# Celebrandil/CudaSift

Hardware: AMD Instinct MI355X
Metric: 1920x1080 SIFT frames/sec (higher is better)
Workload: dtype f32

## Files before the change

cudasift_amd/csrc/common.hpp:

```cpp
#pragma once
#include <hip/hip_runtime.h>
#include <stdint.h>
#include <stddef.h>
#include "misift.h"

#define NUM_SCALES 5
#define NUM_BLURS  8
#define NUM_DOG    7
#define CNT_STRIDE 64
#define CNT_MAXPTS 17
#define CNT_CAND   20
#define CNT_CANDOVF 28
#define CNT_PTOVF  29
#define CNT_CHAINTMO 30
#define CNT_DET    32
#define CNT_DUP    40
#define CNT_SPARE_BLOCKS 9
#define CNT_BIG    48
#define CNT_TICKET 49
#define CNT_ORIDONE 50
#define CNT_FUSETMO 31

struct alignas(16) SiftPointD {
  float xpos, ypos, scale, sharpness, edgeness, orientation, score, ambiguity;
// ... 281 lines not shown
  unsigned int *d_counters;
  unsigned int *h_counters;
  int cap_frames;
  unsigned int *d_cand;
  size_t cand_cap;
  Detection *d_det;
  Detection *d_det_sorted;
  int descr_occ;
  int tile_descr, tile_orient;
  int bin_detections;
  int cap_det_frames, det_max_pts;
  float *d_own_scratch;
  size_t own_scratch_floats;
  int lds_pad_lpd, lds_pad_scan, lds_pad_orient, lds_pad_descr;
  float patch_reach;
  int fold_descr_tail;
  int descr_big_fallbacks;
  PendingBig pending_big;
  unsigned *d_refcap;
  size_t refcap_bytes;
  unsigned *d_capcnt;
  size_t capcnt_bytes;
  int refcap_limit;
  void *d_match_tmp;
  size_t match_tmp_bytes;
  int num_cus;
  int split_tail, in_capture;
  hipStream_t stream2;
  hipEvent_t ev_fork, ev_join;
  int *pack_counts, *pack_offsets;
  SiftPointD *pack_dst;
  int orient_blocks_per_cu;
  int point_blocks_per_cu;
  int strip_waves_per_cu, scan_waves_per_cu;
  int chain_max_frames;
  int chain_embed;
  unsigned chain_wait_ticks;
  int chain_fallbacks;
  int fuse_orient;
  unsigned fuse_wait_ticks;
  int fuse_fallbacks;
  int bin_min_frames;
  int small_frames;
  int lowpass_tile;
  int strip_rows_small;
  int scan_rows_small_coarse;
// ... 25 lines not shown
hipStream_t misift_ctx_result_stream(misift_ctx *ctx);
int misift_ensure_tmp(misift_ctx *ctx, size_t bytes);
int launch_refcap(misift_ctx *ctx, int w, int h, int nframes, int octave);
int launch_descr_big_pending(misift_ctx *ctx);
bool misift_tiny_call(int width, int height, int num_octaves);
int misift_extract_enqueue(misift_ctx *ctx, const void *d_imgs, int src_u8, int nframes, long long frame_stride,
                           int width, int height, int pitch, int num_octaves, float init_blur, float thresh,
                           float lowest_scale, int scale_up, float *d_scratch, SiftPointD *pts, int max_pts);
int misift_extract_sync(misift_ctx *ctx, const void *d_imgs, int src_u8, int nframes, long long frame_stride, int width,
                        int height, int pitch, int num_octaves, float init_blur, float thresh, float lowest_scale,
                        int scale_up, float *d_scratch, SiftPointD *pts, int max_pts, int *num_pts_out);
int launch_export_counts(misift_ctx *ctx, int nframes, int num_octaves, int max_pts, int *counts_out,
                         int *offsets_out);
int launch_pack_records(misift_ctx *ctx, const SiftPointD *pts, int max_pts, int nframes, const int *offsets,
                        SiftPointD *packed);

#define HIP_TRY(expr)                                                                        \
  do {                                                                                       \
    hipError_t e_ = (expr);                                                                  \
    if (e_ != hipSuccess) {                                                                  \
      misift_set_error("%s failed: %s (%s:%d)", #expr, hipGetErrorString(e_), __FILE__, __LINE__); \
      return MISIFT_EHIP;                                                                    \
    }                                                                                        \
  } while (0)

struct LaunchScope {
  misift_ctx *ctx;
  const char *name;
  LaunchScope(misift_ctx *c, const char *n);
  int finish();
// ... 21 lines not shown
int launch_dog_scan(misift_ctx *ctx, const float *base, const StripGeom &g, const LaplaceTaps &taps,
                      float thresh, int octave);
int launch_refine(misift_ctx *ctx, const float *dog, long long dog_frame_stride, const float *base,
                  long long base_frame_stride, const LaplaceTaps *taps, int w, int h, int pitch, int nframes,
                  float thresh, float edge_limit, float factor, float lowest_scale, float subsampling, int octave,
                  SiftPointD *pts, int max_pts);
int launch_orient(misift_ctx *ctx, const float *base, long long base_frame_stride, int w, int h, int pitch,
                  int nframes, int octave, SiftPointD *pts, int max_pts);
int launch_descr(misift_ctx *ctx, const float *base, long long base_frame_stride, int w, int h, int pitch,
                 int nframes, float subsampling, int octave, SiftPointD *pts, int max_pts);
int launch_rescale(misift_ctx *ctx, SiftPointD *pts, int npts, float scale);
int launch_rescale_batch(misift_ctx *ctx, SiftPointD *pts, int max_pts, int nframes, int num_octaves, float scale);
int launch_sort_segments(misift_ctx *ctx, SiftPointD *pts, int max_pts, int nframes, int num_octaves);
int launch_bin_detections(misift_ctx *ctx, const PyramidInfo &P, int max_pts);
int launch_renumber_dups(misift_ctx *ctx, const PyramidInfo &P, int max_pts);
int launch_orient_all(misift_ctx *ctx, const float *scratch, const PyramidInfo &P, SiftPointD *pts, int max_pts);
int launch_orient_descr_fused(misift_ctx *ctx, const float *scratch, const PyramidInfo &P, SiftPointD *pts, int max_pts);
int launch_descr_all(misift_ctx *ctx, const float *scratch, const PyramidInfo &P, SiftPointD *pts, int max_pts,
                     const int *pack_offsets, SiftPointD *pack_dst);
int launch_export_counts_staged(misift_ctx *ctx, int nframes, int num_octaves, int max_pts, int *counts_out,
                                int *offsets_out);
struct ScanAll;
struct ChainGeom;
int launch_dog_scan_all(misift_ctx *ctx, const float *scratch, const PyramidInfo &P, const LaplaceTaps *taps,
                        float thresh, int lev_begin, int lev_end, const ChainGeom *chain = nullptr,
                        const float *k5 = nullptr);
int make_chain_geom(ChainGeom *G, long long frame_stride, const int (*dims)[3], const long long *offs, int nlev, int tile);
int launch_refine_all(misift_ctx *ctx, const float *scratch, const PyramidInfo &P, const LaplaceTaps *taps,
                      float thresh, float edge_limit, float factor, int max_pts);
int launch_match(misift_ctx *ctx, SiftPointD *pts1, int row_begin, int row_count, const SiftPointD *pts2, int n2);
int launch_match_split(misift_ctx *ctx, SiftPointD *pts1, int row_begin, int row_count, const SiftPointD *pts2, int n2,
// ... 29 lines not shown
```

cudasift_amd/csrc/kernels_points.hip:

```cpp
#include "common.hpp"

#define WAVES_PER_BLOCK 4

__device__ __forceinline__ void wave_sync()
{
  __builtin_amdgcn_fence(__ATOMIC_RELEASE, "wavefront");
  __builtin_amdgcn_wave_barrier();
  __builtin_amdgcn_fence(__ATOMIC_ACQUIRE, "wavefront");
}

template <int CTRL, int ROW_MASK>
__device__ __forceinline__ float dpp_f(float v)
{
  return __builtin_bit_cast(float, __builtin_amdgcn_update_dpp(0, __builtin_bit_cast(int, v), CTRL, ROW_MASK, 0xf, false));
}
#define DPP_QUAD_XOR1 0xB1
#define DPP_QUAD_XOR2 0x4E
#define DPP_ROW_HALF_MIRROR 0x141
#define DPP_ROW_MIRROR 0x140
#define DPP_ROW_BCAST15 0x142
#define DPP_ROW_BCAST31 0x143

__device__ __forceinline__ float wave_sum(float v)
{
// ... 1372 lines not shown
  __threadfence_system();
  __syncthreads();
  if (threadIdx.x == 0) __hip_atomic_store(host_out + nwords, host_seq, __ATOMIC_RELEASE, __HIP_MEMORY_SCOPE_SYSTEM);
}
__device__ __forceinline__ bool last_workgroup(unsigned *counters)
{
  __shared__ unsigned s_last;
  asm volatile("s_waitcnt vmcnt(0)" ::: "memory");
  __builtin_amdgcn_fence(__ATOMIC_RELEASE, "workgroup");
  __syncthreads();
  if (threadIdx.x == 0) s_last = atomicAdd(counters + CNT_TICKET, 1u) == gridDim.x * gridDim.y - 1 ? 1u : 0u;
  __syncthreads();
  return s_last != 0;
}

__device__ __forceinline__ bool last_workgroup_2level(unsigned *spare)
{
  __shared__ unsigned s_last2;
  asm volatile("s_waitcnt vmcnt(0)" ::: "memory");
  __builtin_amdgcn_fence(__ATOMIC_RELEASE, "workgroup");
  __syncthreads();
  if (threadIdx.x == 0) {
    const unsigned nwg = gridDim.x * gridDim.y, lb = blockIdx.y * gridDim.x + blockIdx.x;
    const unsigned sub = lb & 15u, members = (nwg - sub + 15u) / 16u;
    unsigned last = 0u;
    if (atomicAdd(&spare[80 + 32 * sub], 1u) == members - 1u) {
      const unsigned nsub = nwg < 16u ? nwg : 16u;
      if (atomicAdd(&spare[48], 1u) == nsub - 1u) last = 1u;
    }
    s_last2 = last;
  }
  __syncthreads();
  return s_last2 != 0;
}

template <bool Q8, int OCC, bool BAL>
__global__ __launch_bounds__(256, OCC) void descr_all_kernel(const float *__restrict__ scratch, PyramidInfo P,
                                                        unsigned *__restrict__ counters,
                                                        const Detection *__restrict__ det,
                                                        SiftPointD *__restrict__ pts, int max_pts, int frac8,
                                                        const int *__restrict__ pack_offsets,
                                                        SiftPointD *__restrict__ pack_dst,
                                                        unsigned *__restrict__ big_list, unsigned big_stride,
                                                        const int4 *__restrict__ block_map,
                                                        unsigned *__restrict__ tail_host_out, unsigned tail_seq)
{
  __shared__ DescrWaveLds s_w[WAVES_PER_BLOCK];
  descr_all_body<Q8, BAL>(scratch, P, counters, det, pts, max_pts, pack_offsets, pack_dst, big_list, big_stride, s_w,
                          block_map);
  if (!BAL && tail_host_out) {
    if (last_workgroup_2level(counters + (size_t)P.nframes * CNT_STRIDE))
      export_counters_host(counters, (unsigned)P.nframes, tail_host_out, tail_seq);
  }
}

template <bool Q8>
__global__ __launch_bounds__(256) void descr_big_kernel(const float *__restrict__ scratch, PyramidInfo P,
                                                        const unsigned *__restrict__ counters,
                                                        const Detection *__restrict__ det,
                                                        SiftPointD *__restrict__ pts, int max_pts,
                                                        const int *__restrict__ pack_offsets,
                                                        SiftPointD *__restrict__ pack_dst,
                                                        const unsigned *__restrict__ big_list, unsigned big_stride,
                                                        unsigned *__restrict__ host_out, unsigned host_seq)
{
  __shared__ __attribute__((aligned(16))) float s_smp[WAVES_PER_BLOCK][DESCR_TBL];
  __shared__ float s_gauss[WAVES_PER_BLOCK][16];
  const int wave = threadIdx.x >> 6, lane = threadIdx.x & 63;
  const int frame = blockIdx.y;
  const unsigned *cnt = counters + (size_t)frame * CNT_STRIDE;
  const unsigned nbig = min(cnt[CNT_BIG], big_stride);
  if (nbig != 0)
    descr_big_frame<Q8>(scratch, P, cnt, det, pts, max_pts, pack_offsets, pack_dst, big_list, big_stride, nbig,
                        s_smp[wave], s_gauss[wave], lane, frame, blockIdx.x * WAVES_PER_BLOCK + wave,
                        gridDim.x * WAVES_PER_BLOCK);
  if (!host_out) return;
  if (!last_workgroup(const_cast<unsigned *>(counters))) return;
  export_counters_host(counters, gridDim.y, host_out, host_seq);
}

template <bool Q8, bool BAL, bool FUSE = false>
__device__ __forceinline__ void orient_gather_body(const float *__restrict__ scratch, const PyramidInfo &P,
                                                   unsigned *__restrict__ counters, Detection *__restrict__ det, int max_pts,
                                                   const int4 *__restrict__ block_map, float *hist, float *gauss, float2 *smp,
                                                   float *tgrid, unsigned *s_done = nullptr, int fuse_items = 0)
{
  const int wave = threadIdx.x >> 6, lane = threadIdx.x & 63;
  const FrameShare fs = frame_share<BAL>(block_map);
  if (BAL && fs.frame < 0) return;
  const int frame = fs.frame;
  unsigned *cnt = counters + (size_t)frame * CNT_STRIDE;
  Detection *fdet = det + (size_t)frame * MISIFT_MAX_OCTAVES * max_pts;
  const bool q8 = Q8;
// ... 19 lines not shown
      d->ori1 = r.ori1;
      d->ori2 = r.ori2;
#ifdef FUSE_NO_DUP_ATOMIC
      d->dupslot = r.has2 ? 0 : -1;
#else
      d->dupslot = r.has2 ? (int)atomicAdd(&cnt[CNT_DUP + co], 1u) : -1;
#endif
      if (FUSE && co < P.noct) atomicAdd(&s_done[co], 1u);
    }
  }
}

#ifndef ORIENT_OCC
#define ORIENT_OCC 6
#endif
template <bool Q8, bool BAL>
__global__ __launch_bounds__(256, ORIENT_OCC) void orient_all_gather_kernel(const float *__restrict__ scratch, PyramidInfo P,
                                                         unsigned *__restrict__ counters,
                                                         Detection *__restrict__ det, int max_pts, int frac8,
                                                         const int4 *__restrict__ block_map)
{
  __shared__ float s_hist[WAVES_PER_BLOCK][64];
  __shared__ float s_gauss[WAVES_PER_BLOCK][16];
  __shared__ float2 s_smp[WAVES_PER_BLOCK][128];
  __shared__ float s_tgrid[WAVES_PER_BLOCK][176];
  const int wave = threadIdx.x >> 6;
  orient_gather_body<Q8, BAL>(scratch, P, counters, det, max_pts, block_map, s_hist[wave], s_gauss[wave], s_smp[wave],
                              s_tgrid[wave]);
}

#ifndef FUSE_POLL_SLEEP
#define FUSE_POLL_SLEEP 32
#endif
#ifndef FUSE_STAMPS
#define FUSE_STAMPS 0
#endif
#if FUSE_STAMPS
__device__ unsigned g_fuse_stamp[16];
#define FUSE_STAMP_MAX(slot) do { if (threadIdx.x == 0) atomicMax(&g_fuse_stamp[slot], (unsigned)wall_clock64()); } while (0)
#define FUSE_STAMP_MIN(slot) do { if (threadIdx.x == 0) atomicMin(&g_fuse_stamp[slot], (unsigned)wall_clock64()); } while (0)
extern "C" int misift_debug_fuse_stamps(unsigned *out16)
{
  unsigned init[16];
// ... 353 lines not shown

static int build_block_maps(misift_ctx *ctx, const PyramidInfo &P, int max_pts)
{
  if (ctx->cur_balanced) return MISIFT_OK;
  bool wanted = false;
  int rc = prepare_block_maps(ctx, P, &wanted);
  if (rc || !wanted) return rc;
  LaunchScope ls(ctx, "frame_shares");
  hipLaunchKernelGGL(frame_shares_kernel, dim3(1), dim3(256), 0, ctx->stream, ctx->d_counters, P.nframes, P.noct, max_pts,
                     ctx->map_t_orient, ctx->d_block_map, ctx->map_t_descr, ctx->d_block_map + ctx->map_t_orient);
  rc = ls.finish();
  if (rc == MISIFT_OK) ctx->cur_balanced = 1;
  return rc;
}

int launch_orient_all(misift_ctx *ctx, const float *scratch, const PyramidInfo &P, SiftPointD *pts, int max_pts)
{
  (void)pts;
  {
    int rc = build_block_maps(ctx, P, max_pts);
    if (rc) return rc;
  }
  LaunchScope ls(ctx, "orient_all");
  Detection *det = ctx->cur_binned ? ctx->d_det_sorted : ctx->d_det;
  const dim3 grid(points_grid_x(ctx, P.nframes, ctx->orient_blocks_per_cu), P.nframes);
  const bool q8 = ctx->opt.texfrac_bits == 8;
  if (ctx->tile_orient) LAUNCH_Q8(orient_all_kernel, grid, dim3(256), scratch, P, ctx->d_counters, det, max_pts, 0);
  else if (ctx->cur_balanced) {
    const dim3 flat(ctx->map_t_orient);
    if (q8) hipLaunchKernelGGL((orient_all_gather_kernel<true, true>), flat, dim3(256), (size_t)ctx->lds_pad_orient, ctx->stream, scratch, P,
                               ctx->d_counters, det, max_pts, 0, ctx->d_block_map);
    else hipLaunchKernelGGL((orient_all_gather_kernel<false, true>), flat, dim3(256), (size_t)ctx->lds_pad_orient, ctx->stream, scratch, P,
                            ctx->d_counters, det, max_pts, 0, ctx->d_block_map);
  } else {
    if (q8) hipLaunchKernelGGL((orient_all_gather_kernel<true, false>), grid, dim3(256), (size_t)ctx->lds_pad_orient, ctx->stream, scratch, P,
                               ctx->d_counters, det, max_pts, 0, (const int4 *)nullptr);
    else hipLaunchKernelGGL((orient_all_gather_kernel<false, false>), grid, dim3(256), (size_t)ctx->lds_pad_orient, ctx->stream, scratch, P,
                            ctx->d_counters, det, max_pts, 0, (const int4 *)nullptr);
  }
  return ls.finish();
}

int launch_descr_all(misift_ctx *ctx, const float *scratch, const PyramidInfo &P, SiftPointD *pts, int max_pts,
                     const int *pack_offsets, SiftPointD *pack_dst)
{
  LaunchScope ls(ctx, "descr_all");
  const Detection *det = ctx->cur_binned ? ctx->d_det_sorted : ctx->d_det;
  const dim3 grid(points_grid_x(ctx, P.nframes), P.nframes);
  if (ctx->tile_descr) {
    unsigned big_stride = 0;
    for (int o = 1; o <= P.noct; o++) big_stride += P.o[o].cand_cap;
    unsigned *host_out = nullptr;
    if (ctx->want_export && !ctx->in_capture) {
// ... 10 lines not shown
                                                 ctx->d_counters, det, pts, max_pts, 0, pack_offsets, pack_dst, ctx->d_cand, \
                                                 big_stride, bmap, tail_out, ctx->export_seq)
#define DESCR_LAUNCH_B(Q, O) do { if (bal) DESCR_LAUNCH(Q, O, true); else DESCR_LAUNCH(Q, O, false); } while (0)
    const bool q8 = ctx->opt.texfrac_bits == 8;
    if (ctx->descr_occ >= 4) { if (q8) DESCR_LAUNCH_B(true, 4); else DESCR_LAUNCH_B(false, 4); }
    else { if (q8) DESCR_LAUNCH_B(true, 3); else DESCR_LAUNCH_B(false, 3); }
#undef DESCR_LAUNCH_B
#undef DESCR_LAUNCH
    PendingBig &pb = ctx->pending_big;
    pb.valid = 0;
    if (fold) {
      pb.valid = 1; pb.scratch = scratch; pb.P = P; pb.det = det; pb.pts = pts; pb.max_pts = max_pts;
      pb.pack_offsets = pack_offsets; pb.pack_dst = pack_dst; pb.big_stride = big_stride;
    } else {
      LAUNCH_Q8(descr_big_kernel, dim3(2, P.nframes), dim3(256), scratch, P, ctx->d_counters, det, pts, max_pts,
                pack_offsets, pack_dst, ctx->d_cand, big_stride, host_out, ctx->export_seq);
    }
  } else
    LAUNCH_Q8(descr_all_gather_kernel, grid, dim3(256), scratch, P, ctx->d_counters, det, pts, max_pts, 0, pack_offsets,
              pack_dst);
  return ls.finish();
}

int launch_orient_descr_fused(misift_ctx *ctx, const float *scratch, const PyramidInfo &P, SiftPointD *pts, int max_pts)
{
  LaunchScope ls(ctx, "orient_descr");
  Detection *det = ctx->d_det;
  const dim3 grid(points_grid_x(ctx, P.nframes), P.nframes);
  unsigned big_stride = 0;
  for (int o = 1; o <= P.noct; o++) big_stride += P.o[o].cand_cap;
  unsigned *host_out = nullptr;
// ... 7 lines not shown
  const bool q8 = ctx->opt.texfrac_bits == 8;
#define FUSED_LAUNCH(Q, O) hipLaunchKernelGGL((orient_descr_fused_kernel<Q, O>), grid, dim3(256), (size_t)ctx->lds_pad_descr, ctx->stream, \
                                              scratch, P, ctx->d_counters, det, pts, max_pts, ctx->d_cand, big_stride,                \
                                              ctx->fuse_wait_ticks, tail_out, ctx->export_seq)
  if (!q8) FUSED_LAUNCH(false, 3);
  else if (ctx->descr_occ >= 4) FUSED_LAUNCH(true, 4);
  else FUSED_LAUNCH(true, 3);
#undef FUSED_LAUNCH
  PendingBig &pb = ctx->pending_big;
  pb.valid = 0;
  if (fold) {
    pb.valid = 1; pb.scratch = scratch; pb.P = P; pb.det = det; pb.pts = pts; pb.max_pts = max_pts;
    pb.pack_offsets = nullptr; pb.pack_dst = nullptr; pb.big_stride = big_stride;
  } else {
    LAUNCH_Q8(descr_big_kernel, dim3(2, P.nframes), dim3(256), scratch, P, ctx->d_counters, det, pts, max_pts,
              (const int *)nullptr, (SiftPointD *)nullptr, ctx->d_cand, big_stride, host_out, ctx->export_seq);
  }
  return ls.finish();
}

int launch_descr_big_pending(misift_ctx *ctx)
{
  PendingBig &pb = ctx->pending_big;
  if (!pb.valid) return MISIFT_OK;
  pb.valid = 0;
  ctx->export_seq++;
  ctx->descr_big_fallbacks++;
  const float *scratch = pb.scratch;
  const PyramidInfo &P = pb.P;
  LaunchScope ls(ctx, "descr_big");
  LAUNCH_Q8(descr_big_kernel, dim3(2, P.nframes), dim3(256), scratch, P, ctx->d_counters, pb.det, pb.pts, pb.max_pts,
            pb.pack_offsets, pb.pack_dst, ctx->d_cand, pb.big_stride, ctx->h_counters, ctx->export_seq);
  return ls.finish();
}

int launch_rescale_batch(misift_ctx *ctx, SiftPointD *pts, int max_pts, int nframes, int num_octaves, float scale)
{
  LaunchScope ls(ctx, "rescale");
  const int slot = 2 * num_octaves + (ctx->opt.fix_numpts ? 1 : 0);
  hipLaunchKernelGGL(rescale_batch_kernel, dim3(16, nframes), dim3(256), 0, ctx->stream, pts, max_pts, ctx->d_counters,
                     slot, scale);
  return ls.finish();
}

int launch_sort_segments(misift_ctx *ctx, SiftPointD *pts, int max_pts, int nframes, int num_octaves)
{
  int rc = misift_ensure_tmp(ctx, sizeof(SiftPointD) * (size_t)nframes * max_pts);
// ... 39 lines not shown
```

cudasift_amd/csrc/misift_host.hip:

```cpp
#include <stdarg.h>
#include <stdio.h>
#include <stdlib.h>
#include <string.h>
#include <math.h>
#include <initializer_list>
#include <map>
#include <mutex>
#include <string>
#include <utility>
#include <vector>
#include "common.hpp"
#include "chain.hpp"
#include "pair_plan.hpp"

static thread_local char g_err[512] = "";

void misift_set_error(const char *fmt, ...)
{
  va_list ap;
  va_start(ap, fmt);
  vsnprintf(g_err, sizeof(g_err), fmt, ap);
  va_end(ap);
}

extern "C" const char *misift_last_error(void) { return g_err; }

// ... 246 lines not shown
  if ((e = getenv("MISIFT_REFERENCE_CAP"))) opt->reference_cap = atoi(e) != 0;
}

struct KnobName { const char *name, *env; };
static const KnobName KNOBS[] = {
  {"graph", "MISIFT_GRAPH"}, {"split_tail", "MISIFT_SPLIT_TAIL"}, {"bin", "MISIFT_BIN"}, {"descr_occ", "MISIFT_DESCR_OCC"},
  {"tile", "MISIFT_TILE"}, {"tile_descr", "MISIFT_TILE_DESCR"}, {"tile_orient", "MISIFT_TILE_ORIENT"},
  {"orient_blocks", "MISIFT_ORIENT_BLOCKS"}, {"point_blocks", "MISIFT_POINT_BLOCKS"}, {"strip_waves", "MISIFT_STRIP_WAVES"},
  {"scan_waves", "MISIFT_SCAN_WAVES"}, {"chain_frames", "MISIFT_CHAIN_FRAMES"}, {"chain_embed", "MISIFT_CHAIN_EMBED"},
  {"chain_wait_us", "MISIFT_CHAIN_WAIT_US"}, {"bin_min_frames", "MISIFT_BIN_MIN_FRAMES"}, {"small_frames", "MISIFT_SMALL_FRAMES"},
  {"balance", "MISIFT_BALANCE"}, {"fold_tail", "MISIFT_FOLD_TAIL"}, {"patch_reach", "MISIFT_TEST_PATCH_REACH"},
  {"lds_pad_lpd", "MISIFT_LDS_PAD_LPD"}, {"lds_pad_scan", "MISIFT_LDS_PAD_SCAN"}, {"lds_pad_orient", "MISIFT_LDS_PAD_ORIENT"},
  {"lds_pad_descr", "MISIFT_LDS_PAD_DESCR"}, {"lowpass_tile", "MISIFT_LOWPASS_TILE"}, {"strip_rows_small", "MISIFT_STRIP_ROWS_SMALL"},
  {"scan_rows_small_coarse", "MISIFT_SCAN_ROWS_SMALL_COARSE"}, {"scan_rows_small", "MISIFT_SCAN_ROWS_SMALL"},
  {"host_spin", "MISIFT_HOST_SPIN"}, {"refcap_limit", "MISIFT_TEST_REFCAP_LIMIT"}, {"fuse_orient", "MISIFT_FUSE_ORIENT"},
  {"fuse_wait_us", "MISIFT_FUSE_WAIT_US"},
};
static bool tunables_from_env()
{
  const char *e = getenv("MISIFT_TUNABLES");
  return e && atoi(e) != 0;
}
static int apply_knob(misift_ctx *ctx, const char *name, double v)
{
  const int i = (int)v;
  const auto is = [&](const char *n) { return strcmp(name, n) == 0; };
  if (is("graph")) extra(ctx)->graph_mode = i != 0;
  else if (is("split_tail")) ctx->split_tail = i;
  else if (is("bin")) ctx->bin_detections = i != 0;
  else if (is("descr_occ")) ctx->descr_occ = i;
  else if (is("tile")) ctx->tile_descr = ctx->tile_orient = i != 0;
// ... 11 lines not shown
  else if (is("balance")) ctx->balance_frames = i != 0;
  else if (is("fold_tail")) ctx->fold_descr_tail = i != 0;
  else if (is("patch_reach")) { if (v > 0.0 && v < 17.9) ctx->patch_reach = (float)v; else if (v >= 17.9) ctx->patch_reach = 17.9f; }
  else if (is("lds_pad_lpd")) ctx->lds_pad_lpd = i;
  else if (is("lds_pad_scan")) ctx->lds_pad_scan = i;
  else if (is("lds_pad_orient")) ctx->lds_pad_orient = i;
  else if (is("lds_pad_descr")) ctx->lds_pad_descr = i;
  else if (is("lowpass_tile")) ctx->lowpass_tile = i != 0;
  else if (is("strip_rows_small")) ctx->strip_rows_small = i >= 2 ? i / 2 * 2 : 6;
  else if (is("scan_rows_small_coarse")) ctx->scan_rows_small_coarse = i > 0 ? i : 2;
  else if (is("scan_rows_small")) ctx->scan_rows_small = i > 0 ? i : 4;
  else if (is("host_spin")) ctx->host_spin = i != 0;
  else if (is("refcap_limit")) ctx->refcap_limit = i >= 0 && i <= 240 ? i : 32;
  else if (is("fuse_orient")) ctx->fuse_orient = i != 0;
  else if (is("fuse_wait_us")) ctx->fuse_wait_ticks = (unsigned)(v * 100.0);
  else { misift_set_error("misift_test_set_knob: unknown knob '%s'", name); return MISIFT_EINVAL; }
  return MISIFT_OK;
}
extern "C" int misift_test_set_knob(misift_ctx *ctx, const char *name, double value);
extern "C" const char *misift_test_knob_names(void)
{
  static std::string all;
  if (all.empty())
    for (const KnobName &k : KNOBS) all += std::string(all.empty() ? "" : ",") + k.name + "=" + k.env;
  return all.c_str();
}

extern "C" void misift_ctx_destroy(misift_ctx *ctx);
static int ctx_init(misift_ctx *ctx, CtxFull *f, int device, void *stream)
{
// ... 14 lines not shown
    HIP_TRY(hipEventCreateWithFlags(&ctx->ev_join, hipEventDisableTiming));
  }
  ctx->bin_detections = 1;
  ctx->descr_occ = 4;
  ctx->tile_descr = 1;
  ctx->tile_orient = 0;
  ctx->orient_blocks_per_cu = 6;
  ctx->point_blocks_per_cu = 8;
  ctx->chain_max_frames = 4;
  ctx->chain_embed = 1;
  ctx->chain_wait_ticks = 10000000u;
  ctx->bin_min_frames = 4;
  ctx->small_frames = 4;
  ctx->balance_frames = 1;
  ctx->fold_descr_tail = 1;
  ctx->fuse_orient = 0;
  ctx->fuse_wait_ticks = 10000000u;
  ctx->patch_reach = 17.9f;
  ctx->refcap_limit = 32;
  ctx->lowpass_tile = 1;
  ctx->strip_rows_small = 6;
  ctx->scan_rows_small_coarse = 2;
  ctx->scan_rows_small = 4;
  ctx->host_spin = 0;
  if (tunables_from_env()) {
    for (const KnobName &k : KNOBS)
      if (const char *e = getenv(k.env)) apply_knob(ctx, k.name, atof(e));
  }
  HIP_TRY(hipEventCreate(&ctx->ev0));
  HIP_TRY(hipEventCreate(&ctx->ev1));
// ... 106 lines not shown
extern "C" int misift_test_set_knob(misift_ctx *ctx, const char *name, double value)
{
  ARG_CHECK(ctx != nullptr && name != nullptr);
  int rc = apply_knob(ctx, name, value);
  if (rc) return rc;
  CtxExtra *x = extra(ctx);
  x->knobs.emplace_back(name, value);
  for (misift_ctx *l : x->lanes) apply_knob(l, name, value);
  return MISIFT_OK;
}

extern "C" int misift_ctx_set_early_return(misift_ctx *ctx, int on)
{
  ARG_CHECK(ctx != nullptr);
  if (!(tunables_from_env() && getenv("MISIFT_HOST_SPIN"))) ctx->host_spin = on ? 1 : 0;
  return MISIFT_OK;
}

extern "C" int misift_ctx_last_call_balanced(misift_ctx *ctx) { return ctx ? ctx->cur_balanced : -1; }

extern "C" int misift_ctx_descr_big_fallbacks(misift_ctx *ctx) { return ctx ? ctx->descr_big_fallbacks : -1; }

extern "C" int misift_ctx_chain_fallbacks(misift_ctx *ctx) { return ctx ? ctx->chain_fallbacks : -1; }
extern "C" int misift_ctx_fuse_fallbacks(misift_ctx *ctx) { return ctx ? ctx->fuse_fallbacks : -1; }

extern "C" int misift_ctx_get_batches_in_flight(misift_ctx *ctx)
{
  return ctx ? (extra(ctx)->lanes.empty() ? 1 : (int)extra(ctx)->lanes.size()) : 0;
}

// ... 716 lines not shown
      rc = launch_dog_scan_all(ctx, d_scratch, P, tapsv.data(), thresh, 0, num_octaves, embedded ? &embed : nullptr, k5);
      if (rc) return rc;
    }
    rc = launch_refine_all(ctx, d_scratch, P, tapsv.data(), thresh, 10.0f, 1.0f / NUM_SCALES, max_pts);
    if (rc) return rc;
    const bool binned = (ctx->bin_detections && nframes >= ctx->bin_min_frames) || ctx->opt.deterministic;
    ctx->cur_binned = binned ? 1 : 0;
    ctx->cur_balanced = 0;
    if (binned) {
      rc = launch_bin_detections(ctx, P, max_pts);
      if (rc) return rc;
    }
    if (ctx->fuse_orient && !binned && !ctx->pack_dst && nframes <= ctx->small_frames && ctx->tile_descr && !ctx->tile_orient &&
        !ctx->in_capture)
      return launch_orient_descr_fused(ctx, d_scratch, P, pts, max_pts);
    rc = launch_orient_all(ctx, d_scratch, P, pts, max_pts);
    if (rc) return rc;
    if (ctx->opt.deterministic) {
      rc = launch_renumber_dups(ctx, P, max_pts);
      if (rc) return rc;
    }
    if (ctx->pack_dst) {
      rc = launch_export_counts_staged(ctx, nframes, num_octaves, max_pts, ctx->pack_counts, ctx->pack_offsets);
      if (rc) return rc;
    }
    return launch_descr_all(ctx, d_scratch, P, pts, max_pts, ctx->pack_offsets, ctx->pack_dst);
  }
  for (int o = 1; o <= num_octaves; o++) {
    const Level &L = lv[o];
    if (L.w < 1 || L.h < 1) continue;
    const float subsampling = (float)(1 << (num_octaves - o));
    const LaplaceTaps taps = octave_taps(table, o);
    {
      StripGeom g = make_geom(ctx, L.w, L.h, L.p, nframes, SS, L.w, L.h, 62);
      rc = launch_laplace(ctx, L.img, g, memoryTmp, SS, taps);
      if (rc) return rc;
      rc = launch_detect(ctx, memoryTmp, g, SS, thresh, o);
// ... 126 lines not shown
  ctx->stream = saved;
  ctx->in_capture = 0;
  const hipError_t e = hipStreamEndCapture(x->gstream, &graph);
  if (rc || e != hipSuccess || !graph || hipGraphInstantiate(&x->gexec, graph, nullptr, nullptr, 0) != hipSuccess) {
    (void)hipGetLastError();
    if (graph) hipGraphDestroy(graph);
    x->gexec = nullptr;
    x->graph_mode = 0;
    return 0;
  }
  hipGraphDestroy(graph);
  x->graph_key = key;
  x->have_graph = true;
  return enqueue_via_graph(ctx, key, d_imgs, frame_stride, d_scratch, pts);
}

struct TinyScope {
  misift_ctx *ctx;
  int saved;
  TinyScope(misift_ctx *c, int w, int h, int noct) : ctx(c), saved(c ? c->opt.fused : 0)
  {
    if (ctx && dense_call(ctx, w, h, noct)) ctx->opt.fused = 0;
  }
  ~TinyScope() { if (ctx) ctx->opt.fused = saved; }
};

int misift_extract_sync(misift_ctx *ctx, const void *d_imgs, int src_u8, int nframes, long long frame_stride, int width,
                        int height, int pitch, int num_octaves, float init_blur, float thresh, float lowest_scale,
                        int scale_up, float *d_scratch, SiftPointD *pts, int max_pts, int *num_pts_out)
{
// ... 133 lines not shown
{
  ARG_CHECK(num_pts_out != nullptr);
  int rc = misift_extract_sync(ctx, d_imgs, 1, nframes, (long long)frame_stride, width, height, pitch, num_octaves,
                        init_blur, thresh, lowest_scale, 0, d_scratch, (SiftPointD *)d_pts, max_pts, num_pts_out);
  if (rc) return rc;
  return resolve_profile(ctx);
}

extern "C" int misift_extract_batch_async(misift_ctx *ctx, const float *d_imgs, int nframes, size_t frame_stride,
                                          int width, int height, int pitch, int num_octaves, float init_blur,
                                          float thresh, float lowest_scale, float *d_scratch, void *d_pts,
                                          int max_pts, int *d_counts_out)
{
  ARG_CHECK(ctx != nullptr);
  TinyScope tiny(ctx, width, height, num_octaves);
  int rc = misift_extract_enqueue(ctx, d_imgs, 0, nframes, (long long)frame_stride, width, height, pitch,
                                  num_octaves, init_blur, thresh, lowest_scale, 0, d_scratch, (SiftPointD *)d_pts,
                                  max_pts);
  if (rc) return rc;
  if (d_counts_out) return launch_export_counts(ctx, nframes, num_octaves, max_pts, d_counts_out, nullptr);
  return MISIFT_OK;
}

extern "C" int misift_extract_batch_packed_async(misift_ctx *ctx, const float *d_imgs, int nframes,
                                                 size_t frame_stride, int width, int height, int pitch,
                                                 int num_octaves, float init_blur, float thresh, float lowest_scale,
                                                 float *d_scratch, void *d_pts, int max_pts, int *d_counts_out,
                                                 int *d_offsets_out, void *d_packed_out)
{
  ARG_CHECK(ctx && d_counts_out && d_offsets_out && d_packed_out);
  TinyScope tiny(ctx, width, height, num_octaves);
  CtxExtra *px = extra(ctx);
  if (!px->lanes.empty()) {
    const size_t k = px->lanes.size();
    misift_ctx *lane = px->lanes[px->ticket % k];
// ... 617 lines not shown
```

cudasift_amd/csrc/pipeline.hip:

```cpp
#include <string.h>
#include <vector>
#include "common.hpp"

__global__ __launch_bounds__(1024) void export_counts_kernel(const unsigned *__restrict__ counters, int nframes, int slot,
                                                              int max_pts, int *__restrict__ counts,
                                                              int *__restrict__ offsets, int staged_noct)
{
  __shared__ int wave_tot[16];
  __shared__ int carry_s;
  const int tid = threadIdx.x, lane = tid & 63, wave = tid >> 6;
  if (tid == 0) carry_s = 0;
  __syncthreads();
  for (int f0 = 0; f0 < nframes; f0 += 1024) {
    const int f = f0 + tid;
    int c = 0;
    if (f < nframes) {
      const unsigned *cnt = counters + (size_t)f * CNT_STRIDE;
      unsigned n = cnt[slot];
      if (staged_noct > 0) {
        n = 0;
        for (int k = 1; k <= staged_noct; k++) {
          n += cnt[CNT_DET + k];
          if (k < staged_noct || (slot & 1)) n += cnt[CNT_DUP + k];
        }
      }
      c = (int)(n < (unsigned)max_pts ? n : (unsigned)max_pts);
      counts[f] = cnt[CNT_CANDOVF] ? -1 : c;
      if (cnt[CNT_CANDOVF]) c = 0;
    }
    if (!offsets) continue;
    int incl = c;
    for (int d = 1; d < 64; d <<= 1) {
      const int o = __shfl_up(incl, d, 64);
      if (lane >= d) incl += o;
    }
    if (lane == 63) wave_tot[wave] = incl;
    __syncthreads();
    int base = carry_s;
    for (int w = 0; w < wave; w++) base += wave_tot[w];
    if (f < nframes) offsets[f] = base + incl - c;
    __syncthreads();
    if (tid == 1023) carry_s = base + incl;
    __syncthreads();
// ... 164 lines not shown
    return MISIFT_EINVAL;
  }
  misift_ctx *ctx = p->ctx;
  HIP_TRY(hipSetDevice(ctx->device));
  PipeSlot &s = p->slots[p->submitted % p->depth];
  const size_t elem = p->src_u8 ? 1 : sizeof(float);
  HIP_TRY(hipMemcpyAsync(s.d_frames, host_frames, elem * p->frame_elems * nframes, hipMemcpyHostToDevice, p->s_up));
  HIP_TRY(hipEventRecord(s.ev_uploaded, p->s_up));
  HIP_TRY(hipStreamWaitEvent(p->s_compute, s.ev_uploaded, 0));
  hipStream_t saved = ctx->stream;
  const int saved_split = ctx->split_tail;
  ctx->stream = p->s_compute;
  ctx->split_tail = 0;
  const int fused_saved = ctx->opt.fused;
  if (misift_tiny_call(p->width, p->height, p->num_octaves)) ctx->opt.fused = 0;
  int rc = misift_extract_enqueue(ctx, s.d_frames, p->src_u8, nframes, (long long)p->frame_elems, p->width, p->height,
                                  p->width, p->num_octaves, p->init_blur, p->thresh, p->lowest_scale, 0, p->d_scratch,
                                  p->d_pts, p->max_pts);
  if (!rc) rc = launch_export_counts(ctx, nframes, p->num_octaves, p->max_pts, s.d_counts, s.d_counts + p->batch);
  if (!rc) rc = launch_pack_records(ctx, p->d_pts, p->max_pts, nframes, s.d_counts + p->batch, s.d_packed);
  ctx->stream = saved;
  ctx->split_tail = saved_split;
  ctx->opt.fused = fused_saved;
  if (rc) return rc;
  HIP_TRY(hipEventRecord(s.ev_done, p->s_compute));
  HIP_TRY(hipStreamWaitEvent(p->s_down, s.ev_done, 0));
  HIP_TRY(hipMemcpyAsync(s.h_counts, s.d_counts, sizeof(int) * (2 * (size_t)p->batch + 1), hipMemcpyDeviceToHost,
                         p->s_down));
  HIP_TRY(hipEventRecord(s.ev_counts, p->s_down));
  s.nframes = nframes;
  p->submitted++;
  return MISIFT_OK;
}

// ... 75 lines not shown
```

Baseline: 58630.

## Fold per-frame count/offset export into last workgroup of orient and descr kernels

Removes the separate export_counts kernel launch by computing per-frame point counts and prefix offsets in the last-finishing workgroup of the orientation-gather kernel (staged case) or the big-descriptor kernel. A two-level ticket counter placed in spare counter words picks the last workgroup, and a single wave then does a shuffle prefix scan. The count logic is moved into a shared helper used by host, test and kernel. This saves one kernel launch per batch, at the cost of a serial single-wave tail and extra atomics in the orient kernel.

```diff
diff --git a/cudasift_amd/csrc/common.hpp b/cudasift_amd/csrc/common.hpp
--- a/cudasift_amd/csrc/common.hpp
+++ b/cudasift_amd/csrc/common.hpp
@@ -319,6 +319,7 @@
   size_t own_scratch_floats;
   int lds_pad_lpd, lds_pad_scan, lds_pad_orient, lds_pad_descr;
   float patch_reach;
+  int pack_tail;
   int fold_descr_tail;
   int descr_big_fallbacks;
   PendingBig pending_big;
@@ -335,6 +336,8 @@
   hipEvent_t ev_fork, ev_join;
   int *pack_counts, *pack_offsets;
   SiftPointD *pack_dst;
+  int *tail_counts, *tail_offsets;
+  int tail_counts_done;
   int orient_blocks_per_cu;
   int point_blocks_per_cu;
   int strip_waves_per_cu, scan_waves_per_cu;
@@ -390,6 +393,13 @@
                          int *offsets_out);
 int launch_pack_records(misift_ctx *ctx, const SiftPointD *pts, int max_pts, int nframes, const int *offsets,
                         SiftPointD *packed);
+
+struct TailCountsScope {
+  misift_ctx *ctx;
+  TailCountsScope(misift_ctx *c, int *counts, int *offsets);
+  ~TailCountsScope();
+  bool done() const;
+};
 
 #define HIP_TRY(expr)                                                                        \
   do {                                                                                       \
@@ -441,7 +451,8 @@
 int launch_sort_segments(misift_ctx *ctx, SiftPointD *pts, int max_pts, int nframes, int num_octaves);
 int launch_bin_detections(misift_ctx *ctx, const PyramidInfo &P, int max_pts);
 int launch_renumber_dups(misift_ctx *ctx, const PyramidInfo &P, int max_pts);
-int launch_orient_all(misift_ctx *ctx, const float *scratch, const PyramidInfo &P, SiftPointD *pts, int max_pts);
+int launch_orient_all(misift_ctx *ctx, const float *scratch, const PyramidInfo &P, SiftPointD *pts, int max_pts,
+                      int *pack_counts = nullptr, int *pack_offsets = nullptr);
 int launch_orient_descr_fused(misift_ctx *ctx, const float *scratch, const PyramidInfo &P, SiftPointD *pts, int max_pts);
 int launch_descr_all(misift_ctx *ctx, const float *scratch, const PyramidInfo &P, SiftPointD *pts, int max_pts,
                      const int *pack_offsets, SiftPointD *pack_dst);
diff --git a/cudasift_amd/csrc/frame_counts.hpp b/cudasift_amd/csrc/frame_counts.hpp
--- /dev/null
+++ b/cudasift_amd/csrc/frame_counts.hpp
@@ -0,0 +1,23 @@
+#pragma once
+#include "common.hpp"
+
+template <class Word>
+__host__ __device__ inline int misift_frame_count(Word word, int num_octaves, int fix_numpts, bool staged, int max_pts,
+                                                  int *width)
+{
+  unsigned n = 0;
+  if (staged) {
+#pragma unroll
+    for (int k = 1; k <= MISIFT_MAX_OCTAVES; k++) {
+      const unsigned nd = word(CNT_DET + k), nu = word(CNT_DUP + k);
+      if (k <= num_octaves) n += nd;
+      if (k < num_octaves || (k == num_octaves && fix_numpts)) n += nu;
+    }
+  } else {
+    n = word(2 * num_octaves + (fix_numpts ? 1 : 0));
+  }
+  const unsigned ovf = word(CNT_CANDOVF);
+  const int c = (int)(n < (unsigned)max_pts ? n : (unsigned)max_pts);
+  *width = ovf ? 0 : c;
+  return ovf ? -1 : c;
+}
diff --git a/cudasift_amd/csrc/kernels_points.hip b/cudasift_amd/csrc/kernels_points.hip
--- a/cudasift_amd/csrc/kernels_points.hip
+++ b/cudasift_amd/csrc/kernels_points.hip
@@ -1,4 +1,5 @@
 #include "common.hpp"
+#include "frame_counts.hpp"
 
 #define WAVES_PER_BLOCK 4
 
@@ -1410,7 +1411,10 @@
   return s_last != 0;
 }
 
-__device__ __forceinline__ bool last_workgroup_2level(unsigned *spare)
+#define TICKET_ORIENT_TOP 56u
+#define TICKET_ORIENT_SUB0 88u
+static_assert(TICKET_ORIENT_SUB0 + 32u * 15u < CNT_SPARE_BLOCKS * CNT_STRIDE, "ticket words lie inside the spare counter blocks");
+__device__ __forceinline__ bool last_workgroup_2level(unsigned *spare, unsigned top = 48u, unsigned sub0 = 80u)
 {
   __shared__ unsigned s_last2;
   asm volatile("s_waitcnt vmcnt(0)" ::: "memory");
@@ -1420,14 +1424,40 @@
     const unsigned nwg = gridDim.x * gridDim.y, lb = blockIdx.y * gridDim.x + blockIdx.x;
     const unsigned sub = lb & 15u, members = (nwg - sub + 15u) / 16u;
     unsigned last = 0u;
-    if (atomicAdd(&spare[80 + 32 * sub], 1u) == members - 1u) {
+    if (atomicAdd(&spare[sub0 + 32 * sub], 1u) == members - 1u) {
       const unsigned nsub = nwg < 16u ? nwg : 16u;
-      if (atomicAdd(&spare[48], 1u) == nsub - 1u) last = 1u;
+      if (atomicAdd(&spare[top], 1u) == nsub - 1u) last = 1u;
     }
     s_last2 = last;
   }
   __syncthreads();
   return s_last2 != 0;
+}
+
+template <bool STAGED>
+__device__ __forceinline__ void frame_counts_tail(const unsigned *counters, int nframes, int noct, int fix_numpts,
+                                                  int max_pts, int *__restrict__ counts, int *__restrict__ offsets)
+{
+  const int lane = threadIdx.x;
+  int carry = 0;
+  for (int f0 = 0; threadIdx.x < 64 && f0 < nframes; f0 += 64) {
+    const int f = f0 + lane;
+    int c = 0;
+    if (f < nframes) {
+      const unsigned *cnt = counters + (size_t)f * CNT_STRIDE;
+      const auto word = [cnt](int i) { return __hip_atomic_load(&cnt[i], __ATOMIC_RELAXED, __HIP_MEMORY_SCOPE_SYSTEM); };
+      counts[f] = misift_frame_count(word, noct, fix_numpts, STAGED, max_pts, &c);
+    }
+    if (!offsets) continue;
+    int incl = c;
+    for (int d = 1; d < 64; d <<= 1) {
+      const int o = __shfl_up(incl, d, 64);
+      if (lane >= d) incl += o;
+    }
+    if (f < nframes) offsets[f] = carry + incl - c;
+    carry += __shfl(incl, 63, 64);
+  }
+  if (offsets && threadIdx.x == 0) offsets[nframes] = carry;
 }
 
 template <bool Q8, int OCC, bool BAL>
@@ -1458,7 +1488,8 @@
                                                         const int *__restrict__ pack_offsets,
                                                         SiftPointD *__restrict__ pack_dst,
                                                         const unsigned *__restrict__ big_list, unsigned big_stride,
-                                                        unsigned *__restrict__ host_out, unsigned host_seq)
+                                                        unsigned *__restrict__ host_out, unsigned host_seq,
+                                                        int *__restrict__ counts_out, int *__restrict__ offsets_out)
 {
   __shared__ __attribute__((aligned(16))) float s_smp[WAVES_PER_BLOCK][DESCR_TBL];
   __shared__ float s_gauss[WAVES_PER_BLOCK][16];
@@ -1470,9 +1501,10 @@
     descr_big_frame<Q8>(scratch, P, cnt, det, pts, max_pts, pack_offsets, pack_dst, big_list, big_stride, nbig,
                         s_smp[wave], s_gauss[wave], lane, frame, blockIdx.x * WAVES_PER_BLOCK + wave,
                         gridDim.x * WAVES_PER_BLOCK);
-  if (!host_out) return;
+  if (!host_out && !counts_out) return;
   if (!last_workgroup(const_cast<unsigned *>(counters))) return;
-  export_counters_host(counters, gridDim.y, host_out, host_seq);
+  if (counts_out) frame_counts_tail<false>(counters, (int)gridDim.y, P.noct, P.fix_numpts, max_pts, counts_out, offsets_out);
+  if (host_out) export_counters_host(counters, gridDim.y, host_out, host_seq);
 }
 
 template <bool Q8, bool BAL, bool FUSE = false>
@@ -1522,11 +1554,12 @@
 #ifndef ORIENT_OCC
 #define ORIENT_OCC 6
 #endif
-template <bool Q8, bool BAL>
+template <bool Q8, bool BAL, bool TAIL>
 __global__ __launch_bounds__(256, ORIENT_OCC) void orient_all_gather_kernel(const float *__restrict__ scratch, PyramidInfo P,
                                                          unsigned *__restrict__ counters,
                                                          Detection *__restrict__ det, int max_pts, int frac8,
-                                                         const int4 *__restrict__ block_map)
+                                                         const int4 *__restrict__ block_map,
+                                                         int *__restrict__ pack_counts, int *__restrict__ pack_offsets)
 {
   __shared__ float s_hist[WAVES_PER_BLOCK][64];
   __shared__ float s_gauss[WAVES_PER_BLOCK][16];
@@ -1535,6 +1568,10 @@
   const int wave = threadIdx.x >> 6;
   orient_gather_body<Q8, BAL>(scratch, P, counters, det, max_pts, block_map, s_hist[wave], s_gauss[wave], s_smp[wave],
                               s_tgrid[wave]);
+  if (TAIL) {
+    if (last_workgroup_2level(counters + (size_t)P.nframes * CNT_STRIDE, TICKET_ORIENT_TOP, TICKET_ORIENT_SUB0))
+      frame_counts_tail<true>(counters, P.nframes, P.noct, P.fix_numpts, max_pts, pack_counts, pack_offsets);
+  }
 }
 
 #ifndef FUSE_POLL_SLEEP
@@ -1918,9 +1955,14 @@
   return rc;
 }
 
-int launch_orient_all(misift_ctx *ctx, const float *scratch, const PyramidInfo &P, SiftPointD *pts, int max_pts)
+int launch_orient_all(misift_ctx *ctx, const float *scratch, const PyramidInfo &P, SiftPointD *pts, int max_pts,
+                      int *pack_counts, int *pack_offsets)
 {
   (void)pts;
+  if ((pack_counts != nullptr) != (pack_offsets != nullptr) || (pack_counts && ctx->tile_orient)) {
+    misift_set_error("launch_orient_all: counts / offsets tail asked of a launch that has none");
+    return MISIFT_EINVAL;
+  }
   {
     int rc = build_block_maps(ctx, P, max_pts);
     if (rc) return rc;
@@ -1931,16 +1973,16 @@
   const bool q8 = ctx->opt.texfrac_bits == 8;
   if (ctx->tile_orient) LAUNCH_Q8(orient_all_kernel, grid, dim3(256), scratch, P, ctx->d_counters, det, max_pts, 0);
   else if (ctx->cur_balanced) {
+#define ORIENT_LAUNCH(Q, B, T, G, MAP) hipLaunchKernelGGL((orient_all_gather_kernel<Q, B, T>), G, dim3(256), (size_t)ctx->lds_pad_orient, \
+                                                         ctx->stream, scratch, P, ctx->d_counters, det, max_pts, 0, MAP, pack_counts,  \
+                                                         pack_offsets)
+#define ORIENT_LAUNCH_T(Q, B, G, MAP) do { if (pack_counts) ORIENT_LAUNCH(Q, B, true, G, MAP); else ORIENT_LAUNCH(Q, B, false, G, MAP); } while (0)
     const dim3 flat(ctx->map_t_orient);
-    if (q8) hipLaunchKernelGGL((orient_all_gather_kernel<true, true>), flat, dim3(256), (size_t)ctx->lds_pad_orient, ctx->stream, scratch, P,
-                               ctx->d_counters, det, max_pts, 0, ctx->d_block_map);
-    else hipLaunchKernelGGL((orient_all_gather_kernel<false, true>), flat, dim3(256), (size_t)ctx->lds_pad_orient, ctx->stream, scratch, P,
-                            ctx->d_counters, det, max_pts, 0, ctx->d_block_map);
+    if (q8) ORIENT_LAUNCH_T(true, true, flat, ctx->d_block_map); else ORIENT_LAUNCH_T(false, true, flat, ctx->d_block_map);
   } else {
-    if (q8) hipLaunchKernelGGL((orient_all_gather_kernel<true, false>), grid, dim3(256), (size_t)ctx->lds_pad_orient, ctx->stream, scratch, P,
-                               ctx->d_counters, det, max_pts, 0, (const int4 *)nullptr);
-    else hipLaunchKernelGGL((orient_all_gather_kernel<false, false>), grid, dim3(256), (size_t)ctx->lds_pad_orient, ctx->stream, scratch, P,
-                            ctx->d_counters, det, max_pts, 0, (const int4 *)nullptr);
+    if (q8) ORIENT_LAUNCH_T(true, false, grid, (const int4 *)nullptr); else ORIENT_LAUNCH_T(false, false, grid, (const int4 *)nullptr);
+#undef ORIENT_LAUNCH_T
+#undef ORIENT_LAUNCH
   }
   return ls.finish();
 }
@@ -1981,7 +2023,8 @@
       pb.pack_offsets = pack_offsets; pb.pack_dst = pack_dst; pb.big_stride = big_stride;
     } else {
       LAUNCH_Q8(descr_big_kernel, dim3(2, P.nframes), dim3(256), scratch, P, ctx->d_counters, det, pts, max_pts,
-                pack_offsets, pack_dst, ctx->d_cand, big_stride, host_out, ctx->export_seq);
+                pack_offsets, pack_dst, ctx->d_cand, big_stride, host_out, ctx->export_seq, ctx->tail_counts, ctx->tail_offsets);
+      if (ctx->tail_counts) ctx->tail_counts_done = 1;
     }
   } else
     LAUNCH_Q8(descr_all_gather_kernel, grid, dim3(256), scratch, P, ctx->d_counters, det, pts, max_pts, 0, pack_offsets,
@@ -2019,7 +2062,9 @@
     pb.pack_offsets = nullptr; pb.pack_dst = nullptr; pb.big_stride = big_stride;
   } else {
     LAUNCH_Q8(descr_big_kernel, dim3(2, P.nframes), dim3(256), scratch, P, ctx->d_counters, det, pts, max_pts,
-              (const int *)nullptr, (SiftPointD *)nullptr, ctx->d_cand, big_stride, host_out, ctx->export_seq);
+              (const int *)nullptr, (SiftPointD *)nullptr, ctx->d_cand, big_stride, host_out, ctx->export_seq, ctx->tail_counts,
+              ctx->tail_offsets);
+    if (ctx->tail_counts) ctx->tail_counts_done = 1;
   }
   return ls.finish();
 }
@@ -2035,7 +2080,8 @@
   const PyramidInfo &P = pb.P;
   LaunchScope ls(ctx, "descr_big");
   LAUNCH_Q8(descr_big_kernel, dim3(2, P.nframes), dim3(256), scratch, P, ctx->d_counters, pb.det, pb.pts, pb.max_pts,
-            pb.pack_offsets, pb.pack_dst, ctx->d_cand, pb.big_stride, ctx->h_counters, ctx->export_seq);
+            pb.pack_offsets, pb.pack_dst, ctx->d_cand, pb.big_stride, ctx->h_counters, ctx->export_seq, (int *)nullptr,
+            (int *)nullptr);
   return ls.finish();
 }
 
diff --git a/cudasift_amd/csrc/misift_host.hip b/cudasift_amd/csrc/misift_host.hip
--- a/cudasift_amd/csrc/misift_host.hip
+++ b/cudasift_amd/csrc/misift_host.hip
@@ -10,6 +10,7 @@
 #include <utility>
 #include <vector>
 #include "common.hpp"
+#include "frame_counts.hpp"
 #include "chain.hpp"
 #include "pair_plan.hpp"
 
@@ -286,7 +287,7 @@
   {"lds_pad_descr", "MISIFT_LDS_PAD_DESCR"}, {"lowpass_tile", "MISIFT_LOWPASS_TILE"}, {"strip_rows_small", "MISIFT_STRIP_ROWS_SMALL"},
   {"scan_rows_small_coarse", "MISIFT_SCAN_ROWS_SMALL_COARSE"}, {"scan_rows_small", "MISIFT_SCAN_ROWS_SMALL"},
   {"host_spin", "MISIFT_HOST_SPIN"}, {"refcap_limit", "MISIFT_TEST_REFCAP_LIMIT"}, {"fuse_orient", "MISIFT_FUSE_ORIENT"},
-  {"fuse_wait_us", "MISIFT_FUSE_WAIT_US"},
+  {"fuse_wait_us", "MISIFT_FUSE_WAIT_US"}, {"pack_tail", "MISIFT_PACK_TAIL"},
 };
 static bool tunables_from_env()
 {
@@ -328,6 +329,7 @@
   else if (is("refcap_limit")) ctx->refcap_limit = i >= 0 && i <= 240 ? i : 32;
   else if (is("fuse_orient")) ctx->fuse_orient = i != 0;
   else if (is("fuse_wait_us")) ctx->fuse_wait_ticks = (unsigned)(v * 100.0);
+  else if (is("pack_tail")) ctx->pack_tail = i != 0;
   else { misift_set_error("misift_test_set_knob: unknown knob '%s'", name); return MISIFT_EINVAL; }
   return MISIFT_OK;
 }
@@ -372,6 +374,7 @@
   ctx->small_frames = 4;
   ctx->balance_frames = 1;
   ctx->fold_descr_tail = 1;
+  ctx->pack_tail = 1;
   ctx->fuse_orient = 0;
   ctx->fuse_wait_ticks = 10000000u;
   ctx->patch_reach = 17.9f;
@@ -508,6 +511,24 @@
 {
   ARG_CHECK(ctx != nullptr);
   if (!(tunables_from_env() && getenv("MISIFT_HOST_SPIN"))) ctx->host_spin = on ? 1 : 0;
+  return MISIFT_OK;
+}
+
+extern "C" int misift_test_packed_counts(const unsigned *counters, int nframes, int num_octaves, int fix_numpts, int max_pts,
+                                         int staged, int *counts, int *offsets)
+{
+  if (!counters || !counts || !offsets || nframes < 1 || num_octaves < 1 || num_octaves > MISIFT_MAX_OCTAVES || max_pts < 1)
+    return MISIFT_EINVAL;
+  int carry = 0;
+  for (int f = 0; f < nframes; f++) {
+    const unsigned *cnt = counters + (size_t)f * CNT_STRIDE;
+    int width = 0;
+    counts[f] = misift_frame_count([cnt](int i) { return cnt[i]; }, num_octaves, fix_numpts ? 1 : 0, staged != 0, max_pts,
+                                   &width);
+    offsets[f] = carry;
+    carry += width;
+  }
+  offsets[nframes] = carry;
   return MISIFT_OK;
 }
 
@@ -1254,13 +1275,15 @@
     if (ctx->fuse_orient && !binned && !ctx->pack_dst && nframes <= ctx->small_frames && ctx->tile_descr && !ctx->tile_orient &&
         !ctx->in_capture)
       return launch_orient_descr_fused(ctx, d_scratch, P, pts, max_pts);
-    rc = launch_orient_all(ctx, d_scratch, P, pts, max_pts);
+    const bool pack_tail = ctx->pack_dst && ctx->pack_tail && !ctx->opt.deterministic && !ctx->tile_orient;
+    rc = launch_orient_all(ctx, d_scratch, P, pts, max_pts, pack_tail ? ctx->pack_counts : nullptr,
+                           pack_tail ? ctx->pack_offsets : nullptr);
     if (rc) return rc;
     if (ctx->opt.deterministic) {
       rc = launch_renumber_dups(ctx, P, max_pts);
       if (rc) return rc;
     }
-    if (ctx->pack_dst) {
+    if (ctx->pack_dst && !pack_tail) {
       rc = launch_export_counts_staged(ctx, nframes, num_octaves, max_pts, ctx->pack_counts, ctx->pack_offsets);
       if (rc) return rc;
     }
@@ -1417,6 +1440,16 @@
   x->have_graph = true;
   return enqueue_via_graph(ctx, key, d_imgs, frame_stride, d_scratch, pts);
 }
+
+TailCountsScope::TailCountsScope(misift_ctx *c, int *counts, int *offsets) : ctx(c)
+{
+  if (ctx) { ctx->tail_counts = ctx->pack_tail ? counts : nullptr; ctx->tail_offsets = ctx->pack_tail ? offsets : nullptr; ctx->tail_counts_done = 0; }
+}
+TailCountsScope::~TailCountsScope()
+{
+  if (ctx) { ctx->tail_counts = nullptr; ctx->tail_offsets = nullptr; ctx->tail_counts_done = 0; }
+}
+bool TailCountsScope::done() const { return ctx && ctx->tail_counts_done != 0; }
 
 struct TinyScope {
   misift_ctx *ctx;
@@ -1580,11 +1613,12 @@
 {
   ARG_CHECK(ctx != nullptr);
   TinyScope tiny(ctx, width, height, num_octaves);
+  TailCountsScope tail(ctx, d_counts_out, nullptr);
   int rc = misift_extract_enqueue(ctx, d_imgs, 0, nframes, (long long)frame_stride, width, height, pitch,
                                   num_octaves, init_blur, thresh, lowest_scale, 0, d_scratch, (SiftPointD *)d_pts,
                                   max_pts);
   if (rc) return rc;
-  if (d_counts_out) return launch_export_counts(ctx, nframes, num_octaves, max_pts, d_counts_out, nullptr);
+  if (d_counts_out && !tail.done()) return launch_export_counts(ctx, nframes, num_octaves, max_pts, d_counts_out, nullptr);
   return MISIFT_OK;
 }
 
diff --git a/cudasift_amd/csrc/pipeline.hip b/cudasift_amd/csrc/pipeline.hip
--- a/cudasift_amd/csrc/pipeline.hip
+++ b/cudasift_amd/csrc/pipeline.hip
@@ -1,6 +1,7 @@
 #include <string.h>
 #include <vector>
 #include "common.hpp"
+#include "frame_counts.hpp"
 
 __global__ __launch_bounds__(1024) void export_counts_kernel(const unsigned *__restrict__ counters, int nframes, int slot,
                                                               int max_pts, int *__restrict__ counts,
@@ -16,17 +17,8 @@
     int c = 0;
     if (f < nframes) {
       const unsigned *cnt = counters + (size_t)f * CNT_STRIDE;
-      unsigned n = cnt[slot];
-      if (staged_noct > 0) {
-        n = 0;
-        for (int k = 1; k <= staged_noct; k++) {
-          n += cnt[CNT_DET + k];
-          if (k < staged_noct || (slot & 1)) n += cnt[CNT_DUP + k];
-        }
-      }
-      c = (int)(n < (unsigned)max_pts ? n : (unsigned)max_pts);
-      counts[f] = cnt[CNT_CANDOVF] ? -1 : c;
-      if (cnt[CNT_CANDOVF]) c = 0;
+      counts[f] = misift_frame_count([cnt](int i) { return cnt[i]; }, staged_noct > 0 ? staged_noct : slot >> 1, slot & 1,
+                                     staged_noct > 0, max_pts, &c);
     }
     if (!offsets) continue;
     int incl = c;
@@ -221,10 +213,15 @@
   ctx->split_tail = 0;
   const int fused_saved = ctx->opt.fused;
   if (misift_tiny_call(p->width, p->height, p->num_octaves)) ctx->opt.fused = 0;
-  int rc = misift_extract_enqueue(ctx, s.d_frames, p->src_u8, nframes, (long long)p->frame_elems, p->width, p->height,
-                                  p->width, p->num_octaves, p->init_blur, p->thresh, p->lowest_scale, 0, p->d_scratch,
-                                  p->d_pts, p->max_pts);
-  if (!rc) rc = launch_export_counts(ctx, nframes, p->num_octaves, p->max_pts, s.d_counts, s.d_counts + p->batch);
+  int rc;
+  {
+    TailCountsScope tail(ctx, s.d_counts, s.d_counts + p->batch);
+    rc = misift_extract_enqueue(ctx, s.d_frames, p->src_u8, nframes, (long long)p->frame_elems, p->width, p->height,
+                                p->width, p->num_octaves, p->init_blur, p->thresh, p->lowest_scale, 0, p->d_scratch,
+                                p->d_pts, p->max_pts);
+    if (!rc && !tail.done())
+      rc = launch_export_counts(ctx, nframes, p->num_octaves, p->max_pts, s.d_counts, s.d_counts + p->batch);
+  }
   if (!rc) rc = launch_pack_records(ctx, p->d_pts, p->max_pts, nframes, s.d_counts + p->batch, s.d_packed);
   ctx->stream = saved;
   ctx->split_tail = saved_split;
```

New measurement: 58570. About the same (-0.1%).
